# AlgoLab/RecGraph

Measured on AMD Instinct MI355X. Metric: aligned reads/sec (-m 8 recombination, 1 kbp reads, 10k-row/32-path graph), higher is better.
Workload: dtype int16

## Files before the change

recgraph_amd/csrc/rg_sweep16.hip:

```cpp
#include <algorithm>
#include <type_traits>

#include "rg_path_kernels.hpp"

namespace rg {

namespace {

constexpr int NEG32 = INT32_MIN / 4;
constexpr int NEG16 = -30000;
constexpr int NEGPAIR = (int)(((unsigned)(NEG16 & 0xffff) << 16) | (unsigned)(NEG16 & 0xffff));
constexpr int ONE2 = 0x00010001;

typedef unsigned u32x4 __attribute__((ext_vector_type(4)));
typedef unsigned u32x2 __attribute__((ext_vector_type(2)));
__device__ __forceinline__ __amdgpu_buffer_rsrc_t uniform_rsrc(const void* base, unsigned bytes) {
    const unsigned long long u = (unsigned long long)base;
    const unsigned lo = (unsigned)__builtin_amdgcn_readfirstlane((int)(unsigned)u), hi = (unsigned)__builtin_amdgcn_readfirstlane((int)(unsigned)(u >> 32));
    void* p = (void*)(((unsigned long long)hi << 32) | lo);
    return __builtin_amdgcn_make_buffer_rsrc(p, 0, (int)__builtin_amdgcn_readfirstlane((int)bytes), 0x00020000);
}
typedef short s16x2 __attribute__((ext_vector_type(2)));
typedef unsigned short u16x2 __attribute__((ext_vector_type(2)));

// ... 18 lines not shown
__device__ __forceinline__ int pk_add_sat(int a, int b) {
    return __builtin_bit_cast(int, __builtin_elementwise_add_sat(__builtin_bit_cast(s16x2, a), __builtin_bit_cast(s16x2, b)));
}
__device__ __forceinline__ int pk_sign(int v) {
    return __builtin_bit_cast(int, (s16x2)(__builtin_bit_cast(s16x2, v) >> (s16x2)(15)));
}
__device__ __forceinline__ int pack16(int lo, int hi) { return (int)(((unsigned)hi << 16) | ((unsigned)lo & 0xffffu)); }
__device__ __forceinline__ int lo16(int v) { return (int)(short)(v & 0xffff); }
__device__ __forceinline__ int hi16(int v) { return v >> 16; }
__device__ __forceinline__ int bfi(int mask, int a, int b) {
    return __builtin_amdgcn_bitop3_b32(mask, a, b, 0xCA);
}

template <int C>
struct RowOps16 {
    static constexpr int H = C / 2;
    static constexpr unsigned FULL = H >= 16 ? 0xffffffffu : ((((1u << H) - 1u) << 16) | ((1u << H) - 1u));

    static __device__ __forceinline__ void alpha(int (&row)[H], const int (&s)[H], int g_i, int g0, int lane, int (&XU)[H], int (&XL)[H], int& lmax) {
        const int GI = pack16(g_i, g_i);
        const int GI0 = lane == 0 ? pack16(g0, g_i) : GI;
        int prev = __builtin_amdgcn_alignbit(row[H - 1], dpp_shr1(row[H - 1], NEGPAIR), 16);
        int m[H];
#pragma unroll
        for (int r = 0; r < H; ++r) {
            const int old = row[r];
            const int d = pk_add(prev, s[r]), u = pk_add(old, r == 0 ? GI0 : GI);
            const int du = pk_max(d, u);
            XU[r] = pk_sub(d, du);
            row[r] = du;
            m[r] = du;
            prev = old;
        }
        static_assert((H & (H - 1)) == 0, "the prefix tree needs a power-of-two register count (m[H - 1] = the lane's maximum)");
#pragma unroll
        for (int w = 1; w < H; w <<= 1) {
#pragma unroll
            for (int r = 2 * w - 1; r < H; r += 2 * w) m[r] = pk_max(m[r - w], m[r]);
        }
        const int run = m[H - 1];
#pragma unroll
        for (int w = H / 4; w >= 1; w >>= 1) {
#pragma unroll
            for (int r = 3 * w - 1; r < H; r += 2 * w) m[r] = pk_max(m[r - w], m[r]);
        }
        const int TL = lo16(run), TH = hi16(run);
        const int ze = dpp_shr1(dpp_incl_max(max(TH, TL), INT32_MIN), INT32_MIN);
        const int bl = max(ze, NEG16);
        const int bh = max(TL, bl);
        const int carry = pack16(bl, bh);
#pragma unroll
        for (int r = 0; r < H; ++r) {
            const int du = row[r];
            const int v = pk_max(m[r], carry);
            XL[r] = pk_sub(du, v);
            row[r] = v;
        }
        lmax = row[H - 1];
    }
    static __device__ __forceinline__ unsigned masks(const int (&XU)[H], const int (&XL)[H], int (&MU)[H], int (&ML)[H]) {
        int al = -1;
#pragma unroll
        for (int r = 0; r < H; ++r) { MU[r] = pk_sign(XU[r]); ML[r] = pk_sign(XL[r]); al &= ML[r]; }
        return (unsigned)al;
    }
    static __device__ __forceinline__ int src_lane(unsigned lall, int lane) {
        const unsigned long long have = __ballot(lall != 0xffffffffu) & ((1ull << lane) - 1ull);
        return have ? 63 - __clzll((long long)have) : 0;
    }
    static __device__ __forceinline__ unsigned sign_bits(const int (&X)[H]) {
        unsigned b = 0;
#pragma unroll
        for (int r = 0; r < H; ++r) b |= ((unsigned)X[r] >> 15 & (unsigned)ONE2) << r;
        return b;
    }
    static __device__ __forceinline__ unsigned dir_word(const int (&XU)[H], const int (&XL)[H]) {
        static_assert(H <= 8, "one byte per flag kind");
        unsigned w = 0;
#pragma unroll
        for (int r = 0; r < H; ++r) {
            const int p = (int)__builtin_amdgcn_perm((unsigned)XL[r], (unsigned)XU[r], 0x07050301u);
            const int sh = r == 0 ? p : (p >> r);
            w = (unsigned)__builtin_amdgcn_bitop3_b32((int)w, sh, (int)(0x80808080u >> r), 0xF8);
        }
        return w;
    }

    static __device__ __forceinline__ void select_steps(int (&SEL)[H], const int (&s)[H], const int (&MU)[H], int g_i, int g0, int lane) {
        const int GI = pack16(g_i, g_i);
        const int GI0 = lane == 0 ? pack16(g0, g_i) : GI;
#pragma unroll
        for (int r = 0; r < H; ++r) SEL[r] = bfi(MU[r], r == 0 ? GI0 : GI, s[r]);
    }

    template <bool kMove = false>
    static __device__ __forceinline__ void member_p1(int (&row)[H], const int (&SEL)[H], const int (&MU)[H], const int (&ML)[H], unsigned lmask,
                                                     int& zl, int& v_lo) {
        int prev = __builtin_amdgcn_alignbit(row[H - 1], dpp_shr1(row[H - 1], NEGPAIR), 16);
        int lastv = NEGPAIR;
#pragma unroll
        for (int r = 0; r < H; ++r) {
            const int old = row[r];
            const int base = kMove ? bfi(MU[r], old, prev) : pk_add(bfi(MU[r], old, prev), SEL[r]);
            row[r] = base;
            lastv = bfi(ML[r], lastv, base);
            prev = old;
        }
        const unsigned nl = ~lmask & FULL;
        const unsigned nl_lo = nl & 0xffffu, nl_hi = nl >> 16;
        v_lo = lo16(lastv);
        const int v_hi = hi16(lastv);
        zl = nl_hi ? v_hi : (nl_lo ? v_lo : NEG32);
    }
    static __device__ __forceinline__ void member_p2(int (&row)[H], const int (&ML)[H], unsigned lmask, int cur, int v_lo) {
        const unsigned nl_lo = ~lmask & FULL & 0xffffu;
        const int bl = max(cur, NEG16);
        const int bh = nl_lo ? max(v_lo, NEG16) : bl;
        int vprev = pack16(bl, bh);
#pragma unroll
        for (int r = 0; r < H; ++r) {
            const int v = bfi(ML[r], vprev, row[r]);
            row[r] = v;
            vprev = v;
        }
    }
    template <bool kMove = false>
    static __device__ __forceinline__ void member(int (&row)[H], const int (&SEL)[H], int lane,
                                                  const int (&MU)[H], const int (&ML)[H], unsigned lmask, int src) {
        int zl, v_lo;
        member_p1<kMove>(row, SEL, MU, ML, lmask, zl, v_lo);
        member_p2(row, ML, lmask, __shfl(zl, src, WAVE), v_lo);
    }
};

template <int K, int KMAX, class F>
__device__ __forceinline__ void run_dispatch_from(F& f, int n) {
    if constexpr (K >= KMAX) f(std::integral_constant<int, (KMAX > 0 ? KMAX : 1)>{});
    else {
        if (n <= K) f(std::integral_constant<int, K>{});
        else run_dispatch_from<K + 1, KMAX>(f, n);
    }
}

}

constexpr int KRUN_REC = RG_SWEEP16_RUN_PATHS;
constexpr int KRUN_M4 = 3;
constexpr int KRUN_32 = 2;
constexpr int sweep16_krun(int C, bool m4, bool rec_nocolmax, bool wide) {
    if (C <= 16) return m4 ? KRUN_M4 : KRUN_REC;
    return (!wide && (rec_nocolmax || m4)) ? KRUN_32 : 0;
}
constexpr int SWEEP16_WAVES = 2;
constexpr bool PROFILE_AHEAD = false;
constexpr int GATHER_PER_MEMBER_ROW = 84;
constexpr int GATHER_PER_ROW = 160;
constexpr int GATHER_PER_MEMBER_RUN = 90;
constexpr int LAYER16_WAVES = 8;
constexpr int LAYER16_PF = 2;

#ifdef RG_SWEEP16_STALLSTAT
#define RG_STALL_BEGIN() const unsigned long long st_b = __builtin_amdgcn_s_memtime()
#define RG_STALL_END(acc) do { __builtin_amdgcn_s_waitcnt(0x0F70); acc += __builtin_amdgcn_s_memtime() - st_b; } while (0)
#else
#define RG_STALL_BEGIN() ((void)0)
#define RG_STALL_END(acc) ((void)0)
#endif

struct PathWords {
    unsigned long long w0, w1, w2, w3;
    __device__ __forceinline__ unsigned long long get(int i) const { return i == 0 ? w0 : (i == 1 ? w1 : (i == 2 ? w2 : w3)); }
    __device__ __forceinline__ void set(int i, unsigned long long v) { if (i == 0) w0 = v; else if (i == 1) w1 = v; else if (i == 2) w2 = v; else w3 = v; }
};

template <int C, int kColmax, bool kRec, bool kWide, bool kSemi>
__global__ __launch_bounds__(64, SWEEP16_WAVES) void k_sweep16(SweepArgs a) {
    static_assert(kColmax == 0 || kColmax == 1, "column maxima with their rows, or none");
    static_assert(!(kColmax == 1 && kRec), "a record sweep tracks no column maxima (k_colmax_rec reads them out of the records): launch_sweep16");
    constexpr int H = C / 2;
    constexpr bool kTrack = kColmax == 1 || kRec;
    constexpr bool kRet = ((kRec && kColmax == 0) || !kTrack) && !kSemi;
    constexpr int NW = kWide ? RG_PW : 1;
    constexpr bool kChain = !kTrack;
    constexpr int KRUN = sweep16_krun(C, !kTrack, kRec && kColmax == 0, kWide);
    static_assert(!(kRec && C <= 16) || KRUN == RG_SWEEP16_RUN_PATHS, "the split step tables (rg_steps.cpp) are built for register runs of RG_SWEEP16_RUN_PATHS paths");
    const int rd = a.order ? a.order[blockIdx.x] : blockIdx.x;
#ifdef RG_SWEEP16_STALLSTAT
    const unsigned long long st_t0 = __builtin_amdgcn_s_memtime();
    unsigned long long st_run = 0, st_nrun = 0, st_gen = 0;
#endif
    const int lane = threadIdx.x;
    const PathGraphDev& g = a.g;
    const int P = g.P;
    const int wpad = C * WAVE;
    const int wrow = H * WAVE;
    ReadState* rs = a.state + rd;
    const long long ro = a.read_off[rd];
    const int n = __builtin_amdgcn_readfirstlane((int)(a.read_off[rd + 1] - ro));
    if (a.bad[rd] || n + 1 > wpad) {
        if (lane == 0 && !a.rev) { rs->status = a.bad[rd] ? ST_BAD_BASE : ST_WOULD_PANIC; }
        return;
    }
    const uint8_t* read = a.reads + ro - 1;
    const bool rev = a.rev;
    const int ncols = rev ? n : n + 1;
    const int GAP = 5;
    extern __shared__ __attribute__((aligned(16))) int lds16[];
    constexpr int EP = kWide ? RG_MAXP : 64;
    constexpr int GTW = C * WAVE > 5 * 64 ? C * WAVE : 5 * 64;
    int* sct = lds16;
    int* endv = lds16 + 64;
    int* endr = endv + EP;
    int* gT = endr + EP;
    int* s2 = gT;
    int* sprof = gT + GTW;
    const int PR_RVL = P, PR_NPROF = P + 1;
    if (lane < 36) sct[lane] = a.sc.t[lane];
    else if (lane < 44) sct[lane] = 0;
    __syncthreads();
    const int gcost = __builtin_amdgcn_readfirstlane(sct[GAP]);
    for (int e = lane; e < 5 * 64; e += WAVE) {
        const int li = e >> 6, cl = e & 7, ch = (e >> 3) & 7;
        s2[e] = (cl < 6 && ch < 6) ? pack16(sct[li * 6 + cl] - gcost, sct[li * 6 + ch] - gcost) : 0;
    }
    int* rows = a.roll + (long long)rd * (P + 2) * wrow;
    const unsigned lane_row_off = (unsigned)lane * (unsigned)(H * sizeof(int));
    const __amdgpu_buffer_rsrc_t rows_rsrc = uniform_rsrc(rows, (unsigned)((P + 2) * wrow) * 4u);
    auto ld_row = [&](int k, int (&dst)[H]) {
        const int so = k * (int)(wrow * sizeof(int));
        if constexpr (H >= 4) {
#pragma unroll
            for (int r4 = 0; r4 < H / 4; ++r4) {
                const u32x4 v = __builtin_amdgcn_raw_buffer_load_b128(rows_rsrc, (int)lane_row_off + 16 * r4, so, 0);
                dst[4 * r4] = (int)v.x; dst[4 * r4 + 1] = (int)v.y; dst[4 * r4 + 2] = (int)v.z; dst[4 * r4 + 3] = (int)v.w;
            }
        } else {
            const u32x2 v = __builtin_amdgcn_raw_buffer_load_b64(rows_rsrc, (int)lane_row_off, so, 0);
            dst[0] = (int)v.x; dst[1] = (int)v.y;
        }
    };
    auto st_row = [&](int k, const int (&src)[H]) {
        const int so = k * (int)(wrow * sizeof(int));
        if constexpr (H >= 4) {
#pragma unroll
            for (int r4 = 0; r4 < H / 4; ++r4) {
                const u32x4 v = {(unsigned)src[4 * r4], (unsigned)src[4 * r4 + 1], (unsigned)src[4 * r4 + 2], (unsigned)src[4 * r4 + 3]};
                __builtin_amdgcn_raw_buffer_store_b128(v, rows_rsrc, (int)lane_row_off + 16 * r4, so, 0);
                asm volatile("s_nop 1" :: "v"(v));
            }
        } else {
            const u32x2 v = {(unsigned)src[0], (unsigned)src[1]};
            __builtin_amdgcn_raw_buffer_store_b64(v, rows_rsrc, (int)lane_row_off, so, 0);
        }
    };
    unsigned long long pcode[(H + 7) / 8] = {};
    int thrk[(kRec || !kTrack) ? 1 : C];
#define THRK(q) thrk[(kRec || !kTrack) ? 0 : (q)]
    int thz[kRec ? H : 1];
    int minplain2 = 0;
    int thzmin = 0;
    int next_eval = INT32_MAX;
    int minthrk = INT32_MAX;
    int minplain = INT32_MAX;
    const bool tight = a.thr != nullptr || a.oob;
    const int oob = max((int)((float)(n + 1) * (1.0f - a.rbw) / 2.0f), 1);
    auto thr_key = [&](int q, bool member_rule) -> int {
        const int c = lane * C + q;
        const int j = rev ? n - c : c;
        int th = INT32_MAX;
        if (c < ncols && j >= oob && j < n + 1 - oob) {
            if (a.thr) th = a.thr[(long long)rd * wpad + j];
            else if (a.lb) th = a.lb[rd] + a.brc - (n - j) * a.maxmatch;
        }
        if (th == INT32_MAX) return INT32_MAX;
        long long tz = (long long)th - (long long)c * gcost;
        if (tz > 32767) return INT32_MAX;
        int key = tz < -32768 ? INT32_MIN : (int)tz * 65536;
        if (member_rule) key = max(key, (-c * gcost) * 65536 + 1);
        return key;
    };
    {
#pragma unroll
        for (int q = 0; q < C; ++q) {
            const int c = lane * C + q;
            int code = 4;
            if (c >= 1 && c < ncols) code = rev ? read[n - c + 1] : read[c];
            const int r = q % H, hi = q / H;
            pcode[r / 8] |= (unsigned long long)code << (8 * (r % 8) + 3 * hi);
            if (!kRec && kTrack) THRK(q) = thr_key(q, true);
        }
#pragma unroll
        for (int li = 0; li < 4; ++li) {
#pragma unroll
            for (int r = 0; r < H; ++r) sprof[(li * WAVE + lane) * H + r] = s2[li * 64 + (int)((pcode[r / 8] >> (8 * (r % 8))) & 63)];
        }
        {
            int np[H];
#pragma unroll
            for (int r = 0; r < H; ++r) np[r] = s2[4 * 64 + (int)((pcode[r / 8] >> (8 * (r % 8))) & 63)];
            st_row(PR_NPROF, np);
        }
#pragma unroll
        for (int q = 0; q < (kTrack ? C : 0); ++q) { minthrk = min(minthrk, thr_key(q, true)); minplain = min(minplain, thr_key(q, false)); }
#pragma unroll
        for (int r = 0; r < (kRec ? H : 1); ++r)
            thz[kRec ? r : 0] = pack16(thr_key(kRec ? r : 0, true) >> 16, thr_key(kRec ? r + H : 0, true) >> 16);
        minplain2 = pack16(minplain >> 16, minplain >> 16);
// ... 496 lines not shown
                it.w.set(ka >> 6, it.w.get(ka >> 6) & ~(1ull << (ka & 63)));
                int nx[H];
                int kn = it.next();
                if (kn >= 0) ld_row(kn, nx);
                while (kn >= 0) {
                    const int k = kn;
                    int cur[H];
#pragma unroll
                    for (int r = 0; r < H; ++r) cur[r] = nx[r];
                    kn = it.next();
                    if (kn >= 0) ld_row(kn, nx);
                    int kk = k;
                    asm volatile("" : "+v"(kk));
                    const int K2 = (int)(((unsigned)kk << 16) | (unsigned)kk);
#pragma unroll
                    for (int r = 0; r < H; ++r) {
                        const int d = pk_sub_sat(cur[r], A[r]);
                        const int lt = pk_sign(pk_sub_sat(d, bd[r]));
                        bd[r] = pk_max(bd[r], d);
                        bk[r] = bfi(lt, bk[r], K2);
                    }
                }
#pragma unroll
                for (int r = 0; r < H; ++r) {
                    gT[r * WAVE + lane] = (int)(((unsigned)bd[r] << 16) | ((unsigned)bk[r] & 0xffffu));
                    gT[(r + H) * WAVE + lane] = (int)(((unsigned)bd[r] & 0xffff0000u) | ((unsigned)bk[r] >> 16));
                }
            }
            {
                int gl = lane;
                asm volatile("" : "+v"(gl));
#pragma unroll
                for (int r = 0; r < H; ++r) { const int w = r * WAVE + gl; G[r] = pack16(2 * w, 2 * w + 1); }
            }
            __syncthreads();
            int ri = i, rli = li, rslot = slot, rw1 = w1;
            for (int step = 0;; ++step) {
                const int g_i = gcost;
                const int g0 = kSemi ? 0 : g_i;
                int s[H], MU[H], ML[H], XU[H], XL[H];
                load_steps(rli, s);
                int lmax_unused;
                RowOps16<C>::alpha(A, s, g_i, g0, lane, XU, XL, lmax_unused);
                const bool gdirs = kWide ? ((kColmax == 0 || dirs != nullptr) && (wide_sel || edge_row(ri))) : want_dirs(gmask, 0, ri);
                if (gdirs) store_dirs(rslot, XU, XL);
                const unsigned lmask = RowOps16<C>::masks(XU, XL, MU, ML);
                const int src = RowOps16<C>::src_lane(lmask, lane);
                RowOps16<C>::template member<true>(G, MU, lane, MU, ML, lmask, src);
                cells += (unsigned long long)g_nm;
                done += 2ull;
                if (kRec && track) {
                    int bv[H], K2[H];
                    constexpr int HS = 31 - __builtin_clz(H * WAVE);
#pragma unroll
                    for (int r = 0; r < H; ++r) {
                        const int c0 = G[r] & 0xffff, c1 = (unsigned)G[r] >> 16;
                        const unsigned t0 = (unsigned)gT[(c0 >> 1) + ((c0 & 1) << HS)];
                        const unsigned t1 = (unsigned)gT[(c1 >> 1) + ((c1 & 1) << HS)];
                        bv[r] = pk_add(A[r], (int)__builtin_amdgcn_perm(t1, t0, 0x07060302u));
                        K2[r] = (int)__builtin_amdgcn_perm(t1, t0, 0x05040100u);
                    }
                    const int knm_row = ((rw1 >> 20) & 511) - 1;
                    int acc = -1;
                    if (knm_row >= 0) {
#pragma unroll
                        for (int r = 0; r < H; ++r) acc &= pk_sub_sat(bv[r], thz[kRec ? r : 0]);
                    } else {
#pragma unroll
                        for (int r = 0; r < H; ++r) acc &= pk_sub_sat(bv[r], minplain2);
                    }
                    const bool lhit = ((unsigned)acc & 0x80008000u) != 0x80008000u;
                    if (__any(lhit)) {
                        bool mine;
                        int4* rp = rec_slot(ri, lhit, mine);
                        int hk[H];
#pragma unroll
                        for (int r = 0; r < H; ++r) hk[r] = (int)(((unsigned)bv[r] << 16) | ((unsigned)K2[r] & 0xffffu));
                        rec_half(rp, mine, 0, hk);
#pragma unroll
                        for (int r = 0; r < H; ++r) hk[r] = (int)(((unsigned)bv[r] & 0xffff0000u) | ((unsigned)K2[r] >> 16));
                        rec_half(rp, mine, 1, hk);
                    }
                }
                t += kWide ? went : 1;
                if (step + 1 >= R || t >= nsteps) break;
                int nw0, nw1;
                unsigned long long ngm;
                fetch(t, nw0, nw1, ngm);
                ri = nw0 & 0xfffff; rli = (nw0 >> 20) & 7; rslot = nw1 & 0xfffff; rw1 = nw1;
            }
            done += (unsigned long long)(g_nme - 1) * ((kRec && track) ? 2ull : 1ull);
            {
                int B[H];
                int* gS = gT;
                {
                    int a0[H];
                    ld_row(ka, a0);
                    __syncthreads();
#pragma unroll
                    for (int r = 0; r < H; ++r) gS[r * WAVE + lane] = a0[r];
                    __syncthreads();
                }
#pragma unroll
                for (int r = 0; r < H; ++r) {
                    const int c0 = G[r] & 0xffff, c1 = (unsigned)G[r] >> 16;
                    const int w0v = gS[c0 >> 1], w1v = gS[c1 >> 1];
                    const int a0 = (c0 & 1) ? hi16(w0v) : lo16(w0v), a1 = (c1 & 1) ? hi16(w1v) : lo16(w1v);
                    B[r] = pk_sub_sat(A[r], pack16(a0, a1));
                }
                st_row(ka, A);
                MemberIter it{kWide ? wide_gw : PathWords{gm, 0ull, 0ull, 0ull}, 0};
                it.w.set(ka >> 6, it.w.get(ka >> 6) & ~(1ull << (ka & 63)));
                int nx[H];
                int kn = it.next();
                if (kn >= 0) ld_row(kn, nx);
                while (kn >= 0) {
                    const int k = kn;
                    __syncthreads();
#pragma unroll
                    for (int r = 0; r < H; ++r) gS[r * WAVE + lane] = nx[r];
                    kn = it.next();
                    if (kn >= 0) ld_row(kn, nx);
                    __syncthreads();
                    int outr[H];
#pragma unroll
                    for (int r = 0; r < H; ++r) {
                        const int c0 = G[r] & 0xffff, c1 = (unsigned)G[r] >> 16;
                        const int w0v = gS[c0 >> 1], w1v = gS[c1 >> 1];
                        const int v0 = (c0 & 1) ? hi16(w0v) : lo16(w0v), v1 = (c1 & 1) ? hi16(w1v) : lo16(w1v);
                        outr[r] = pk_add(B[r], pack16(v0, v1));
                    }
                    st_row(k, outr);
                }
            }
            continue;
        }
        int e_i = i, e_w1 = w1, e_flags = flags;
        bool e_adv = true;
        if (kWide && went > 1) e_flags &= ~F_LAST;
        if (kWide ? wide_run : (KRUN > 0 && (flags & F_INNER) && (nm <= KRUN || (kRet && nme <= KRUN && a.gather_ok && !semi_end &&
                                                             run_left * (GATHER_PER_MEMBER_ROW * (nm - 1) - GATHER_PER_ROW) >= GATHER_PER_MEMBER_RUN * (nm - 1))) && run_left > 0)) {
            int rnm = kWide ? wide_n : nme;
            unsigned long long rgm = gmask;
            int mk[KRUN > 0 ? KRUN : 1];
            if (kWide) {
#pragma unroll
                for (int kk = 0; kk < KRUN; ++kk) mk[kk] = wide_ids[kk];
            } else {
                unsigned long long tm = kRet ? gm : rgm;
#pragma unroll
                for (int kk = 0; kk < KRUN; ++kk) { mk[kk] = tm ? kbase + __builtin_ctzll(tm) : 0; tm = tm ? (tm & (tm - 1)) : 0; }
            }
            int rr[KRUN > 0 ? KRUN : 1][H];
#pragma unroll
            for (int kk = 0; kk < KRUN; ++kk)
                if (kk < rnm) ld_row(mk[kk], rr[kk]);
            {
                RG_STALL_BEGIN();
                __builtin_amdgcn_s_waitcnt(0x0F70);
#if defined(RG_SWEEP16_STALLSTAT) && RG_SWEEP16_STALLSTAT == 1
                RG_STALL_END(st_run); ++st_nrun;
#endif
            }
#if defined(RG_SWEEP16_STALLSTAT) && RG_SWEEP16_STALLSTAT == 3
            const unsigned long long st_rb = __builtin_amdgcn_s_memtime();
#endif
            int ri = i, rli = li, rslot = slot, rw1 = w1, rfl = 7;
            int rleft = run_left;
            bool tail = false;
            constexpr bool kAhead = PROFILE_AHEAD && C <= 16;
            int s[H];
            if (kAhead) load_steps(rli, s);
            for (;;) {
            tail = false; rfl = 7;
            auto run_rows = [&](auto rn_tag, auto lean_tag) __attribute__((always_inline)) {
            constexpr int RN = decltype(rn_tag)::value;
            constexpr bool kLean = decltype(lean_tag)::value;
            const unsigned long long run_sel = kWide ? (wide_sel ? ~0ull : 0ull) : rgm;
            const int run_page = 0;
            unsigned nrows = 0;
            while (true) {
                const int g_i = gcost;
                const int g0 = kSemi ? 0 : g_i;
                int XU[H], XL[H];
#if defined(RG_SWEEP16_STALLSTAT) && RG_SWEEP16_STALLSTAT == 3
                ++st_nrun;
#endif
                if (!kAhead) load_steps(rli, s);
                int lmax;
                RowOps16<C>::alpha(rr[0], s, g_i, g0, lane, XU, XL, lmax);
                if constexpr (!kLean) {
                    if (kWide ? ((kColmax == 0 || dirs != nullptr) && (wide_sel || edge_row(ri))) : want_dirs(run_sel, run_page, ri)) store_dirs(rslot, XU, XL);
                }
                if constexpr (RN > 1) {
                    int MU[H], ML[H];
                    const unsigned lmask = RowOps16<C>::masks(XU, XL, MU, ML);
                    const int src = RowOps16<C>::src_lane(lmask, lane);
                    int SEL[H];
                    RowOps16<C>::select_steps(SEL, s, MU, g_i, g0, lane);
                    int zl[KRUN > 0 ? KRUN : 1], vlo[KRUN > 0 ? KRUN : 1];
#pragma unroll
                    for (int kk = 1; kk < KRUN; ++kk)
                        if (kk < RN) { RowOps16<C>::member_p1(rr[kk], SEL, MU, ML, lmask, zl[kk], vlo[kk]); zl[kk] = __shfl(zl[kk], src, WAVE); }
#pragma unroll
                    for (int kk = 1; kk < KRUN; ++kk)
                        if (kk < RN) RowOps16<C>::member_p2(rr[kk], ML, lmask, zl[kk], vlo[kk]);
                }
                if (kAhead && !tail && rleft > 1) {
                    const int tn = t + 1;
                    if ((tn >> 6) != blk) to_block(tn >> 6);
                    load_steps((__builtin_amdgcn_readlane(recs.x, tn & (WAVE - 1)) >> 20) & 7, s);
                }
                ++nrows;
                if (kRec && kColmax == 0 && tail) {
                    if (track) {
                        if (rfl & F_FIRST) row_open = false;
                        int key[C];
                        if (row_open) { keys_ld(key); fold_keys(key, rr[0], mk[0]); } else set_keys(key, rr[0], mk[0]);
#pragma unroll
                        for (int kk = 1; kk < KRUN; ++kk) if (kk < RN) fold_keys(key, rr[kk], mk[kk]);
                        row_open = true;
                        if (rfl & F_LAST) { row_end(ri, ((rw1 >> 20) & 511) - 1, key); row_open = false; }
                        else keys_st(key);
                    }
                } else if constexpr (kLean) {
                } else if (track && kRec && kColmax == 0) {
                    int bv[H];
#pragma unroll
                    for (int r = 0; r < H; ++r) bv[r] = rr[0][r];
#pragma unroll
                    for (int kk = 1; kk < KRUN; ++kk)
                        if (kk < RN) {
#pragma unroll
                            for (int r = 0; r < H; ++r) bv[r] = pk_max(bv[r], rr[kk][r]);
                        }
                    const int knm_row = ((rw1 >> 20) & 511) - 1;
                    int acc = -1;
                    bool fine = true;
                    if constexpr (RN == 1 && kRec) {
                        if (knm_row >= 0) fine = __any(((unsigned)pk_sub_sat(lmax, thzmin) & 0x80008000u) != 0x80008000u);
                    }
                    if (!fine) {
                    } else if (knm_row >= 0) [[likely]] {
#pragma unroll
                        for (int r = 0; r < H; ++r) acc &= pk_sub_sat(bv[r], thz[kRec ? r : 0]);
                    } else {
                        int m = bv[0];
#pragma unroll
                        for (int r = 1; r < H; ++r) m = pk_max(m, bv[r]);
                        acc = pk_sub_sat(m, minplain2);
                    }
                    const bool lhit = ((unsigned)acc & 0x80008000u) != 0x80008000u;
                    if (__any(lhit)) {
                        bool mine;
                        int4* rp = rec_slot(ri, lhit, mine);
#pragma unroll
                        for (int half = 0; half < 2; ++half) {
                            int hk[H];
#pragma unroll
                            for (int kk = 0; kk < KRUN; ++kk)
                                if (kk < RN) {
                                    int kv = mk[kk];
                                    asm volatile("" : "+v"(kv));
#pragma unroll
                                    for (int r = 0; r < H; ++r) {
                                        const int key = half == 0 ? (int)(((unsigned)rr[kk][r] << 16) | (unsigned)kv)
                                                                  : (int)(((unsigned)rr[kk][r] & 0xffff0000u) | (unsigned)kv);
                                        hk[r] = kk == 0 ? key : max(hk[r], key);
                                    }
                                }
                            rec_half(rp, mine, half, hk);
                        }
                    }
                } else if (track) {
                    int key[C];
                    set_keys(key, rr[0], mk[0]);
#pragma unroll
                    for (int kk = 1; kk < KRUN; ++kk) if (kk < RN) fold_keys(key, rr[kk], mk[kk]);
                    row_end(ri, ((rw1 >> 20) & 511) - 1, key);
                }
                if (semi_end) {
#pragma unroll
                    for (int kk = 0; kk < KRUN; ++kk) if (kk < RN) end_fold(mk[kk], ri, rr[kk]);
                    end_row_done(ri);
                }
                t += kWide ? went : 1;
                if (tail || t >= nsteps) break;
                if (rleft > 1) {
                    if ((t >> 6) != blk) to_block(t >> 6);
                    if constexpr (kLean) {
                        const int nw0 = __builtin_amdgcn_readlane(recs.x, t & (WAVE - 1));
                        rli = (nw0 >> 20) & 7;
                        rleft = (nw0 >> 26) & 63;
                        continue;
                    }
                    const int nw0 = __builtin_amdgcn_readlane(recs.x, t & (WAVE - 1)), nw1 = __builtin_amdgcn_readlane(recs.y, t & (WAVE - 1));
                    ri = nw0 & 0xfffff; rli = (nw0 >> 20) & 7; rslot = nw1 & 0xfffff; rw1 = nw1;
                    rleft = (nw0 >> 26) & 63;
                    continue;
                }
                const int pw = peek_w0(t);
                const int nf = (pw >> 23) & 7;
                const bool to_tail = kRec && kColmax == 0 && (nf & F_INNER) && ((pw >> 26) & 63) == 0;
                if (!to_tail && (nf != 7 || ((pw >> 26) & 63) == 0)) break;
                if (peek_gm(t) != rgm) break;
                int nw0, nw1;
                unsigned long long ngm;
                fetch(t, nw0, nw1, ngm);
                ri = nw0 & 0xfffff; rli = (nw0 >> 20) & 7; rslot = nw1 & 0xfffff; rw1 = nw1;
                tail = to_tail; rfl = nf;
                rleft = to_tail ? 0 : (nw0 >> 26) & 63;
                if (kAhead) load_steps(rli, s);
            }
            cells += (unsigned long long)nrows * (unsigned long long)(kWide ? wide_total : __popcll(rgm));
            done += (unsigned long long)nrows * (unsigned long long)RN;
            if constexpr (kSilent) {
                sil[3] += (int)nrows;
                if constexpr (kLean) sil[2] += (int)(nrows - (tail ? 1u : 0u));
            }
            };
            auto run_rows_full = [&](auto rn_tag) __attribute__((always_inline)) { run_rows(rn_tag, std::false_type{}); };
            if constexpr (kSilent) {
                static_assert(!kChain, "a chained run would need the members, row and knm of ITS first record");
                const unsigned long long silent = ((unsigned long long)(unsigned)__builtin_amdgcn_readfirstlane(sil[1]) << 32) | (unsigned)__builtin_amdgcn_readfirstlane(sil[0]);
                const bool lean = (gm & ~silent) == 0ull && (rgm & dsel_w.w0) == 0ull && !edge_row(i) && ((w1 >> 20) & 511) != 0;
                auto run_rows_lean = [&](auto rn_tag) __attribute__((always_inline)) { run_rows(rn_tag, std::true_type{}); };
                if (lean) run_dispatch_from<1, (KRUN > 0 ? KRUN : 1)>(run_rows_lean, rnm);
                else run_dispatch_from<1, (KRUN > 0 ? KRUN : 1)>(run_rows_full, rnm);
            } else
            run_dispatch_from<1, (KRUN > 0 ? KRUN : 1)>(run_rows_full, rnm);
            if (tail) {
                if (semi_end && (rfl & F_LAST)) end_row_done(ri);
                if (rfl & F_LAST) row_open = false;
            }
            bool chain = false;
            unsigned long long gm2 = 0;
            if (kChain && !kWide && !semi_end && t < nsteps && (!kRet || next_eval == INT32_MAX)) {
                const int pw = peek_w0(t);
                if ((((pw >> 23) & 7) & F_INNER) && ((pw >> 26) & 63) != 0) {
                    gm2 = peek_gm(t);
                    chain = __popcll(gm2) <= KRUN && (gm2 & rgm) == 0;
                }
            }
            if (!chain) break;
            int rn[KRUN > 0 ? KRUN : 1][H];
            int mk2[KRUN > 0 ? KRUN : 1];
            {
                unsigned long long tm = gm2;
#pragma unroll
                for (int kk = 0; kk < KRUN; ++kk) { mk2[kk] = tm ? kbase + __builtin_ctzll(tm) : 0; tm = tm ? (tm & (tm - 1)) : 0; }
#pragma unroll
                for (int kk = 0; kk < KRUN; ++kk)
                    if (kk < __popcll(gm2)) ld_row(mk2[kk], rn[kk]);
            }
            __builtin_amdgcn_s_waitcnt(0x0F70);
#pragma unroll
            for (int kk = 0; kk < KRUN; ++kk)
                if (kk < rnm) st_row(mk[kk], rr[kk]);
            rnm = __popcll(gm2);
            rgm = gm2;
#pragma unroll
            for (int kk = 0; kk < KRUN; ++kk) {
                mk[kk] = mk2[kk];
#pragma unroll
                for (int r = 0; r < H; ++r) rr[kk][r] = rn[kk][r];
            }
            {
                int nw0, nw1;
                unsigned long long ngm;
                fetch(t, nw0, nw1, ngm);
                ri = nw0 & 0xfffff; rli = (nw0 >> 20) & 7; rslot = nw1 & 0xfffff; rw1 = nw1;
                rleft = (nw0 >> 26) & 63;
                if (kAhead) load_steps(rli, s);
            }
            }
#pragma unroll
            for (int kk = 0; kk < KRUN; ++kk)
                if (kk < rnm) st_row(mk[kk], rr[kk]);
#if defined(RG_SWEEP16_STALLSTAT) && RG_SWEEP16_STALLSTAT == 3
            st_gen += __builtin_amdgcn_s_memtime() - st_rb;
#endif
            continue;
        } else {
        const int g_i = gcost;
        const int g0 = kSemi ? 0 : g_i;
        int s[H];
        load_steps(li, s);
        int MUl[kWide ? 1 : H], MLl[kWide ? 1 : H];
        unsigned lmaskl = 0;
        int srcl = 0;
        int (&MU)[H] = *reinterpret_cast<int (*)[H]>(kWide ? MUw : MUl);
        int (&ML)[H] = *reinterpret_cast<int (*)[H]>(kWide ? MLw : MLl);
        unsigned& lmask = kWide ? lmaskw : lmaskl;
        int& src = kWide ? srcw : srcl;
        {
            unsigned long long rest = cont ? gm : gm & ~(1ull << (ga - kbase));
            cells += (unsigned long long)nm;
            done += (unsigned long long)nme;
            int nxt[H];
            int knext = -1;
            if (rest) {
                knext = kbase + __builtin_ctzll(rest);
                rest &= rest - 1;
                ld_row(knext, nxt);
            }
            int key[C];
            bool have = false;
            if (track) {
                if (flags & F_FIRST) row_open = false;
                have = row_open;
                if (have) keys_ld(key);
            }
            if (!cont) {
                int rowa[H];
                ld_row(ga, rowa);
#if defined(RG_SWEEP16_STALLSTAT) && RG_SWEEP16_STALLSTAT == 1
                { RG_STALL_BEGIN(); RG_STALL_END(st_gen); }
#endif
                int XU[H], XL[H];
                int lmax_unused;
                RowOps16<C>::alpha(rowa, s, g_i, g0, lane, XU, XL, lmax_unused);
                st_row(ga, rowa);
                bool wd = want_dirs(gmask, page, i);
                if (kWide && !wd && t + 1 < nsteps) wd = peek_w1(t + 1) < 0;
                if (wd) store_dirs(slot, XU, XL);
                lmask = RowOps16<C>::masks(XU, XL, MU, ML);
                src = RowOps16<C>::src_lane(lmask, lane);
                if (track) {
                    if (!have) set_keys(key, rowa, ga); else fold_keys(key, rowa, ga);
                    have = true;
                }
                if (semi_end) end_fold(ga, i, rowa);
            }
            int SEL[H];
            RowOps16<C>::select_steps(SEL, s, MU, g_i, g0, lane);
            while (knext >= 0) {
                const int k = knext;
                int cur[H];
#pragma unroll
                for (int r = 0; r < H; ++r) cur[r] = nxt[r];
                if (rest) {
                    knext = kbase + __builtin_ctzll(rest);
                    rest &= rest - 1;
                    ld_row(knext, nxt);
                } else knext = -1;
                RowOps16<C>::member(cur, SEL, lane, MU, ML, lmask, src);
                st_row(k, cur);
                if (track) fold_keys(key, cur, k);
                if (semi_end) end_fold(k, i, cur);
            }
            if (track) {
                row_open = true;
                if (e_flags & F_LAST) row_end(e_i, ((e_w1 >> 20) & 511) - 1, key);
                else keys_st(key);
            }
        }
        }
        if (semi_end && (e_flags & F_LAST)) end_row_done(e_i);
        if (e_flags & F_LAST) row_open = false;
        if (e_adv) ++t;
    }

    if (kColmax == 1 && a.colmax_out) {
#pragma unroll
        for (int q = 0; q < C; ++q) {
            const int c = lane * C + q;
            if (c < ncols) {
                a.colmax_out[(long long)rd * wpad + (rev ? n - c : c)] = ckey[kColmax == 1 ? q : 0] == INT32_MIN ? NEG32 : (ckey[kColmax == 1 ? q : 0] >> 16) + c * gcost;
                if (a.colarg_out) a.colarg_out[(long long)rd * wpad + (rev ? n - c : c)] = (crow[kColmax == 1 ? q : 0] << 8) | (ckey[kColmax == 1 ? q : 0] & 255);
            }
        }
    }
    if (a.ncand_out && lane == 0) a.ncand_out[rd] = ncand;
    __syncthreads();
    if (!rev && !kSemi) {
        const int ql = n % C, ln = n / C;
        for (int k = lane; k < P; k += WAVE) {
            const int pv = rows[(long long)k * wrow + ln * H + (ql % H)];
            rs->sink_val[k] = (kRet && !((word_of(needed, k >> 6) >> (k & 63)) & 1ull)) ? NEG32 : (ql >= H ? hi16(pv) : lo16(pv)) + n * gcost;
        }
    }
    if (semi_end) {
        for (int k = lane; k < P; k += WAVE) { rs->sink_val[k] = endv[k]; rs->path_end_row[k] = endr[k]; }
        if (lane == ln_end) { rs->s0 = gbest_val; rs->end_row_best = gbest_row; rs->seed_path = gbest_path; }
    }
    if constexpr (kSilent) {
        if (lane == 0 && a.runstat) { atomicAdd(a.runstat, (unsigned)sil[2]); atomicAdd(a.runstat + 1, (unsigned)sil[3]); }
    }
    if (lane == 0 && a.count_cells) {
        const unsigned long long all = kRet && a.table_members ? a.table_members : cells;
#ifdef RG_SWEEP16_STALLSTAT
        {
            const unsigned long long tot = __builtin_amdgcn_s_memtime() - st_t0;
            atomicAdd(a.cells, (tot >> 8) | ((st_gen >> 8) << 32));
            atomicAdd(a.cells + 1, (st_run >> 8) | (st_nrun << 32));
            return;
        }
#endif
#ifdef RG_SWEEP16_RETSTAT
        if (kRet) { atomicAdd(a.cells, stat_e | (stat_n << 32)); atomicAdd(a.cells + 1, stat_h | ((unsigned long long)(rev ? 0 : 1) << 48)); return; }
#endif
        atomicAdd(a.cells, all * (unsigned long long)(n + 1));
        atomicAdd(a.cells + 1, done * (unsigned long long)(n + 1));
    }
}

template <int C>
__global__ __launch_bounds__(256) void k_expand(ExpandArgs a) {
    const int rd = blockIdx.x;
    const int lane = threadIdx.x & (WAVE - 1), wv = threadIdx.x / WAVE, nwv = blockDim.x / WAVE;
    ReadState* rs = a.state + rd;
    if (rs->status & (ST_BAD_BASE | ST_WOULD_PANIC)) return;
    const unsigned nrec = a.nrec[rd];
    if (nrec > a.frec_cap) { if (threadIdx.x == 0) rs->status |= ST_OVERFLOW; return; }
    const int bound = rs->bound;
    const int nread = (int)(a.read_off[rd + 1] - a.read_off[rd]);
    const int oob = max((int)((float)(nread + 1) * (1.0f - a.rbw) / 2.0f), 1);
    const int* base = a.frec + (long long)rd * a.frec_cap * (4 + C);
    Cand* out = a.fcand + (long long)rd * a.fcap;
    const int* wr = a.wr + (long long)rd * a.wpad;
    constexpr int LPR = C / 4, RPW = WAVE / LPR;
    const int part = lane % LPR, sub = lane / LPR;
    for (unsigned t0 = wv * RPW; t0 < nrec; t0 += nwv * RPW) {
        const unsigned t = t0 + sub;
        if (t >= nrec) continue;
        const int* rp = base + (long long)t * (4 + C);
        const int rl = rp[0];
        const int4 k4 = *reinterpret_cast<const int4*>(rp + 4 + 4 * part);
        const int keys[4] = {k4.x, k4.y, k4.z, k4.w};
        const int knm = a.knm[rl >> 6];
#pragma unroll
// ... 378 lines not shown
```

Measured before the change: 131,600.

## Batch run rows per 64-record block and move row loads inside dispatched run body

Restructures the run loop for the non-wide path so it processes a batch of consecutive records within the current 64-record block using readlane on the already-loaded records. This avoids the per-row peek/fetch/to_block checks. Member row loads and stores move inside the compile-time RN-specialized body, so the unroll count matches the actual member count. It also removes the disabled PROFILE_AHEAD step-prefetch path and pins the tail row indices in SGPRs for the lean variant. The rewritten continuation logic, which checks the previous record's run_left and the group mask, adds control-flow complexity and risks subtle mismatches with the old run-termination semantics.

Result: faster. 151,900, median of 6 (+15.5%).

```diff
diff --git a/recgraph_amd/csrc/rg_sweep16.hip b/recgraph_amd/csrc/rg_sweep16.hip
--- a/recgraph_amd/csrc/rg_sweep16.hip
+++ b/recgraph_amd/csrc/rg_sweep16.hip
@@ -194,7 +194,6 @@
     return (!wide && (rec_nocolmax || m4)) ? KRUN_32 : 0;
 }
 constexpr int SWEEP16_WAVES = 2;
-constexpr bool PROFILE_AHEAD = false;
 constexpr int GATHER_PER_MEMBER_ROW = 84;
 constexpr int GATHER_PER_ROW = 160;
 constexpr int GATHER_PER_MEMBER_RUN = 90;
@@ -997,25 +996,29 @@
                 for (int kk = 0; kk < KRUN; ++kk) { mk[kk] = tm ? kbase + __builtin_ctzll(tm) : 0; tm = tm ? (tm & (tm - 1)) : 0; }
             }
             int rr[KRUN > 0 ? KRUN : 1][H];
-#pragma unroll
-            for (int kk = 0; kk < KRUN; ++kk)
-                if (kk < rnm) ld_row(mk[kk], rr[kk]);
-            {
+            auto ld_run = [&](int nrun) {
+#pragma unroll
+                for (int kk = 0; kk < KRUN; ++kk)
+                    if (kk < nrun) ld_row(mk[kk], rr[kk]);
                 RG_STALL_BEGIN();
                 __builtin_amdgcn_s_waitcnt(0x0F70);
 #if defined(RG_SWEEP16_STALLSTAT) && RG_SWEEP16_STALLSTAT == 1
                 RG_STALL_END(st_run); ++st_nrun;
 #endif
-            }
+            };
+            auto st_run = [&](int nrun) {
+#pragma unroll
+                for (int kk = 0; kk < KRUN; ++kk)
+                    if (kk < nrun) st_row(mk[kk], rr[kk]);
+            };
+            constexpr bool kRowsInBody = !kChain && !kWide;
+            if constexpr (!kRowsInBody) ld_run(rnm);
 #if defined(RG_SWEEP16_STALLSTAT) && RG_SWEEP16_STALLSTAT == 3
             const unsigned long long st_rb = __builtin_amdgcn_s_memtime();
 #endif
             int ri = i, rli = li, rslot = slot, rw1 = w1, rfl = 7;
             int rleft = run_left;
             bool tail = false;
-            constexpr bool kAhead = PROFILE_AHEAD && C <= 16;
-            int s[H];
-            if (kAhead) load_steps(rli, s);
             for (;;) {
             tail = false; rfl = 7;
             auto run_rows = [&](auto rn_tag, auto lean_tag) __attribute__((always_inline)) {
@@ -1023,15 +1026,24 @@
             constexpr bool kLean = decltype(lean_tag)::value;
             const unsigned long long run_sel = kWide ? (wide_sel ? ~0ull : 0ull) : rgm;
             const int run_page = 0;
+            if constexpr (kRowsInBody) ld_run(RN);
             unsigned nrows = 0;
             while (true) {
+                int cnt = 1;
+                if constexpr (!kWide) {
+                    if (!tail) cnt = max(min(min(rleft, WAVE - (t & (WAVE - 1))), nsteps - t), 1);
+                }
+                nrows += (unsigned)cnt;
+                int idx = t & (WAVE - 1);
+                for (int left = cnt;;) {
                 const int g_i = gcost;
                 const int g0 = kSemi ? 0 : g_i;
                 int XU[H], XL[H];
 #if defined(RG_SWEEP16_STALLSTAT) && RG_SWEEP16_STALLSTAT == 3
                 ++st_nrun;
 #endif
-                if (!kAhead) load_steps(rli, s);
+                int s[H];
+                load_steps(rli, s);
                 int lmax;
                 RowOps16<C>::alpha(rr[0], s, g_i, g0, lane, XU, XL, lmax);
                 if constexpr (!kLean) {
@@ -1051,12 +1063,6 @@
                     for (int kk = 1; kk < KRUN; ++kk)
                         if (kk < RN) RowOps16<C>::member_p2(rr[kk], ML, lmask, zl[kk], vlo[kk]);
                 }
-                if (kAhead && !tail && rleft > 1) {
-                    const int tn = t + 1;
-                    if ((tn >> 6) != blk) to_block(tn >> 6);
-                    load_steps((__builtin_amdgcn_readlane(recs.x, tn & (WAVE - 1)) >> 20) & 7, s);
-                }
-                ++nrows;
                 if (kRec && kColmax == 0 && tail) {
                     if (track) {
                         if (rfl & F_FIRST) row_open = false;
@@ -1065,7 +1071,9 @@
 #pragma unroll
                         for (int kk = 1; kk < KRUN; ++kk) if (kk < RN) fold_keys(key, rr[kk], mk[kk]);
                         row_open = true;
-                        if (rfl & F_LAST) { row_end(ri, ((rw1 >> 20) & 511) - 1, key); row_open = false; }
+                        int tri = ri, tw1 = rw1;
+                        if constexpr (kLean) asm volatile("" : "+s"(tri), "+s"(tw1));
+                        if (rfl & F_LAST) { row_end(tri, ((tw1 >> 20) & 511) - 1, key); row_open = false; }
                         else keys_st(key);
                     }
                 } else if constexpr (kLean) {
@@ -1129,33 +1137,55 @@
                     for (int kk = 0; kk < KRUN; ++kk) if (kk < RN) end_fold(mk[kk], ri, rr[kk]);
                     end_row_done(ri);
                 }
-                t += kWide ? went : 1;
+                if (--left == 0) break;
+                ++idx;
+                const int nw0 = __builtin_amdgcn_readlane(recs.x, idx);
+                rli = (nw0 >> 20) & 7;
+                if constexpr (!kLean) {
+                    const int nw1 = __builtin_amdgcn_readlane(recs.y, idx);
+                    ri = nw0 & 0xfffff; rslot = nw1 & 0xfffff; rw1 = nw1;
+                }
+                }
+                t += kWide ? went : cnt;
                 if (tail || t >= nsteps) break;
-                if (rleft > 1) {
-                    if ((t >> 6) != blk) to_block(t >> 6);
-                    if constexpr (kLean) {
-                        const int nw0 = __builtin_amdgcn_readlane(recs.x, t & (WAVE - 1));
-                        rli = (nw0 >> 20) & 7;
+                if constexpr (kWide) {
+                    if (rleft > 1) {
+                        if ((t >> 6) != blk) to_block(t >> 6);
+                        const int nw0 = __builtin_amdgcn_readlane(recs.x, t & (WAVE - 1)), nw1 = __builtin_amdgcn_readlane(recs.y, t & (WAVE - 1));
+                        ri = nw0 & 0xfffff; rli = (nw0 >> 20) & 7; rslot = nw1 & 0xfffff; rw1 = nw1;
                         rleft = (nw0 >> 26) & 63;
                         continue;
                     }
-                    const int nw0 = __builtin_amdgcn_readlane(recs.x, t & (WAVE - 1)), nw1 = __builtin_amdgcn_readlane(recs.y, t & (WAVE - 1));
+                    const int pw = peek_w0(t);
+                    const int nf = (pw >> 23) & 7;
+                    const bool to_tail = kRec && kColmax == 0 && (nf & F_INNER) && ((pw >> 26) & 63) == 0;
+                    if (!to_tail && (nf != 7 || ((pw >> 26) & 63) == 0)) break;
+                    if (peek_gm(t) != rgm) break;
+                    int nw0, nw1;
+                    unsigned long long ngm;
+                    fetch(t, nw0, nw1, ngm);
                     ri = nw0 & 0xfffff; rli = (nw0 >> 20) & 7; rslot = nw1 & 0xfffff; rw1 = nw1;
-                    rleft = (nw0 >> 26) & 63;
-                    continue;
-                }
-                const int pw = peek_w0(t);
-                const int nf = (pw >> 23) & 7;
-                const bool to_tail = kRec && kColmax == 0 && (nf & F_INNER) && ((pw >> 26) & 63) == 0;
-                if (!to_tail && (nf != 7 || ((pw >> 26) & 63) == 0)) break;
-                if (peek_gm(t) != rgm) break;
-                int nw0, nw1;
-                unsigned long long ngm;
-                fetch(t, nw0, nw1, ngm);
-                ri = nw0 & 0xfffff; rli = (nw0 >> 20) & 7; rslot = nw1 & 0xfffff; rw1 = nw1;
-                tail = to_tail; rfl = nf;
-                rleft = to_tail ? 0 : (nw0 >> 26) & 63;
-                if (kAhead) load_steps(rli, s);
+                    tail = to_tail; rfl = nf;
+                    rleft = to_tail ? 0 : (nw0 >> 26) & 63;
+                } else {
+                const int last = (__builtin_amdgcn_readlane(recs.x, (t - 1) & (WAVE - 1)) >> 26) & 63;
+                const int nw0 = peek_w0(t);
+                const int nf = (nw0 >> 23) & 7, nfield = (nw0 >> 26) & 63;
+                const bool to_tail = kRec && kColmax == 0 && last <= 1 && (nf & F_INNER) && nfield == 0;
+                if (last <= 1) {
+                    if (!to_tail && (nf != 7 || nfield == 0)) break;
+                    const int idt = t & (WAVE - 1);
+                    if ((((unsigned long long)(unsigned)__builtin_amdgcn_readlane(recs.w, idt) << 32) | (unsigned)__builtin_amdgcn_readlane(recs.z, idt)) != rgm) break;
+                    rfl = nf;
+                }
+                rli = (nw0 >> 20) & 7;
+                tail = to_tail;
+                rleft = nfield;
+                if (!kLean || to_tail) {
+                    const int nw1 = __builtin_amdgcn_readlane(recs.y, t & (WAVE - 1));
+                    ri = nw0 & 0xfffff; rslot = nw1 & 0xfffff; rw1 = nw1;
+                }
+                }
             }
             cells += (unsigned long long)nrows * (unsigned long long)(kWide ? wide_total : __popcll(rgm));
             done += (unsigned long long)nrows * (unsigned long long)RN;
@@ -1163,6 +1193,7 @@
                 sil[3] += (int)nrows;
                 if constexpr (kLean) sil[2] += (int)(nrows - (tail ? 1u : 0u));
             }
+            if constexpr (kRowsInBody) st_run(RN);
             };
             auto run_rows_full = [&](auto rn_tag) __attribute__((always_inline)) { run_rows(rn_tag, std::false_type{}); };
             if constexpr (kSilent) {
@@ -1199,9 +1230,7 @@
                     if (kk < __popcll(gm2)) ld_row(mk2[kk], rn[kk]);
             }
             __builtin_amdgcn_s_waitcnt(0x0F70);
-#pragma unroll
-            for (int kk = 0; kk < KRUN; ++kk)
-                if (kk < rnm) st_row(mk[kk], rr[kk]);
+            st_run(rnm);
             rnm = __popcll(gm2);
             rgm = gm2;
 #pragma unroll
@@ -1216,12 +1245,9 @@
                 fetch(t, nw0, nw1, ngm);
                 ri = nw0 & 0xfffff; rli = (nw0 >> 20) & 7; rslot = nw1 & 0xfffff; rw1 = nw1;
                 rleft = (nw0 >> 26) & 63;
-                if (kAhead) load_steps(rli, s);
-            }
-            }
-#pragma unroll
-            for (int kk = 0; kk < KRUN; ++kk)
-                if (kk < rnm) st_row(mk[kk], rr[kk]);
+            }
+            }
+            if constexpr (!kRowsInBody) st_run(rnm);
 #if defined(RG_SWEEP16_STALLSTAT) && RG_SWEEP16_STALLSTAT == 3
             st_gen += __builtin_amdgcn_s_memtime() - st_rb;
 #endif
```
